# ReactiveBayes/RxInfer.jl

Hardware: AMD Instinct MI355X
Metric: node-message-updates/sec (d=4 LGSSM, T=100k, BP sweep with Bethe free energy) (higher is better)
Workload: dtype f64; 1 GPU; LGSSM d=4 dy=4 T=100000, 1024 independent chains per GPU (BASELINE config 2), 1 BP sweep + Bethe free energy per step; chain c drawn from numpy default_rng(42+c); chains_per_gpu=1024, T=100000, segments=128, segment_len=782

## Files before the change

rxinfer.jl_amd/csrc/engine.hpp:

```cpp
#pragma once
#include <hip/hip_runtime.h>

#include <cstdarg>
#include <cstdint>
#include <cstdio>
#include <initializer_list>
#include <string>
#include <vector>

#include "../../include/rxhip.h"
#include "lgssm_plan.hpp"
#include "tree_engine.hpp"

namespace rxhip {
struct LgssmVtbl;
struct DenseModel;
}
struct DenseTables;
using rxhip::DenseModel;
using rxhip::LgssmVtbl;

struct rxhip_engine_life {
    bool have_data = false;
    long long stream_k = 0;
// ... 118 lines not shown
        long long N = 0;
        int K = 0, KT = 0, materialize = 0, nblocks = 0, it = 0, iterations = 0, hist_cap = 0;
        int mvd = 0;
        int nq = 0;
        int hist_stride = 0;
        int state_size = 0;
        double *d_resp = nullptr, *d_par = nullptr, *d_drv = nullptr, *d_prior = nullptr, *d_init = nullptr,
               *d_partial = nullptr, *d_totals = nullptr, *d_hist = nullptr, *d_fe = nullptr;
    } g;
    bool dense = false;
    int nt = 0;
    double *d_scanm = nullptr, *d_fstart_m = nullptr, *d_beta_xi = nullptr, *d_vend = nullptr, *d_qtab = nullptr, *d_loc = nullptr, *d_bnd = nullptr;
    const int* d_canon = nullptr;
    int scan_sg = 1, scan_ng = 1;
    int agg_oc = 1, agg_kc = 1;
    double* d_aggpart = nullptr;
    bool fused = false;
    double *d_ftab = nullptr, *d_mtab = nullptr, *d_ntab = nullptr, *d_pos = nullptr, *d_fseg = nullptr;
    double fe_const = 0.0;
    double *d_gtab = nullptr, *d_segend = nullptr, *d_sblk = nullptr;
    int ck_log2 = 0;
    int sweep_waves_fwd = 1, sweep_waves_bwd = 1;
    long long nck = 0;
    double *d_amp = nullptr, *d_ainv = nullptr;
    int* d_ckfail = nullptr;
    hipEvent_t ev_tab0 = nullptr, ev_tab1 = nullptr;
    bool sequential = false;
    double* d_elemx = nullptr;
    double* h_io = nullptr;
    size_t h_io_bytes = 0;
    double* h_stream = nullptr;
    double* d_stream = nullptr;
    double *d_mu = nullptr, *d_nu = nullptr, *d_cx = nullptr, *d_cy_raw = nullptr;
    std::vector<double> h_mu, h_nu, h_cx, h_cy, h_offA, h_offB;
    std::vector<double> h_cx_const, h_cy_const;
    std::vector<int> h_offsm;
    int du = 0;
    std::vector<double> h_Bu;
    std::vector<char> h_umask;
    bool off_chain = false;
    double* d_off_chain = nullptr;
    std::vector<double> h_user;
    double* d_user = nullptr;
    int* d_step_model = nullptr;
    bool split = false, split_ready = false;
    int m_dpad = 0, m_nt = 0;
    int m_sg = 0, m_ng = 0;
// ... 131 lines not shown
```

rxinfer.jl_amd/csrc/launch_tables.hpp:

```cpp
#pragma once
#include <hip/hip_runtime.h>

#include <cstdlib>

#include "lgssm_kernels.hpp"
#include "predict_kernels.hpp"
#include "noise_kernels.hpp"
#ifndef RXHIP_LAUNCH_LGSSM_ONLY
#include "dense_kernels.hpp"
#include "dense_tab_kernels.hpp"
#include "dense_mseg_kernels.hpp"
#include "dense_split_kernels.hpp"
#include "dense8_kernels.hpp"
#endif

#ifndef RXHIP_TAB_SAME_TOL
#define RXHIP_TAB_SAME_TOL 5e-15
#endif

namespace rxhip {

struct SweepArgs {
    bool rev;
    int bnd;
    bool write_cov;
    int y_ring;
    int waves;
};
struct LgssmVtbl {
    int d, dy;
    int cst_size, tab_size, agg_size;
    int oA, oP, oLOBS, oG, oQI, oC0, oM1, oV1, oHF;
    int tK, tU;
    int aPI, aC, aJ, aCI, aX, aJJ;
    int scan_size, sM1, sM2, sVB, sN1, sN2, sLB;
    int f0_size, fK, fU, fSI, pos_size, pPI, pJ, pC, fs_size, fsA1, fsA2, fsW, mt_row;
    void (*forward0)(const Params&, const double*, bool, bool, int, hipStream_t);
    void (*time_tables)(const TimeTabParams&, hipStream_t);
    void (*fe_seg)(const Params&, hipStream_t);
    int gt_row, se_size;
    void (*smooth_tables)(const SmoothTabParams&, const double*, hipStream_t);
    void (*backward_sh)(const Params&, const double*, const double* gtab, const double* segend, const SweepArgs&, hipStream_t);
    void (*boundary_scan_tab)(const Params&, const double*, bool, hipStream_t);
    void (*seg_aggregate)(const Params&, const double*, bool, hipStream_t);
    int ex_size;
    void (*seg_elements)(const Params&, hipStream_t);
    void (*boundary_scan)(const Params&, const double*, bool, bool, hipStream_t);
    void (*forward)(const Params&, const double*, bool, bool, hipStream_t);
    void (*backward)(const Params&, const double*, bool, hipStream_t);
    void (*forecast)(const PredictParams&, hipStream_t);
    void (*predict)(const PredictParams&, hipStream_t);
    void (*joint)(const PredictParams&, hipStream_t);
    void (*stream_step)(const StreamParams&, hipStream_t);
    void (*small_sweep)(const Params&, const double*, bool, hipStream_t);
    int noise_prior_size;
    void (*noise_reset)(const NoiseParams&, hipStream_t);
    void (*noise_update)(const NoiseParams&, hipStream_t);
};
void lgssm_vtbls_d1(LgssmVtbl* out);
void lgssm_vtbls_d2(LgssmVtbl* out);
void lgssm_vtbls_d3(LgssmVtbl* out);
void lgssm_vtbls_d4(LgssmVtbl* out);

// ... 38 lines not shown
```

rxinfer.jl_amd/csrc/lgssm_kernels.hpp:

```cpp
#pragma once
#include <hip/hip_runtime.h>
#include <stdint.h>

namespace rxhip {

constexpr int ST_NOT_POSDEF = 1;
constexpr int ST_NONFINITE = 2;
__device__ __forceinline__ void lds_barrier() {
    __builtin_amdgcn_fence(__ATOMIC_RELEASE, "workgroup", "local");
    __builtin_amdgcn_s_barrier();
    __builtin_amdgcn_fence(__ATOMIC_ACQUIRE, "workgroup", "local");
}
__device__ __forceinline__ bool is_finite(double x) { return (__double2hiint(x) & 0x7ff00000) != 0x7ff00000; }

#ifndef RXHIP_NT_STORES
#define RXHIP_NT_STORES 0
#endif
typedef double rx_d2v __attribute__((ext_vector_type(2)));
__device__ __forceinline__ void stream_store(double2* p, double a, double b) {
#if RXHIP_NT_STORES
    rx_d2v v = {a, b};
    __builtin_nontemporal_store(v, reinterpret_cast<rx_d2v*>(p));
#else
    *p = make_double2(a, b);
// ... 152 lines not shown
    double* beta;
    double* fe_part;
    double* fe_chain;
    double* fe_total;
    int iteration;
    int filter;
    double fe_scale;
    int* status;
    int masked;
    const double* ftab;
    const double* mtab;
    const double* ntab;
    const double* fseg;
    double fe_const;
    double* elemx;
    const int* step_model;
    const double* noise_B;
    double* noise_part;
    int skip_marginals;
    int tinv_records;
    int elem_full;
    int ck_log2;
    long long nck;
    const double* ainv;
};


__device__ __forceinline__ double rcp_pos(double x) {
    double r = __builtin_amdgcn_rcp(x);
    double e = __builtin_fma(-x, r, 1.0);
    r = __builtin_fma(r, e, r);
    e = __builtin_fma(-x, r, 1.0);
    r = __builtin_fma(r, e, r);
    return r;
}

template <int D>
__device__ __forceinline__ bool spd_inv(const Sym<D>& a, Sym<D>& out, double& det) {
    double L[D][D], W[D][D], r[D];
    bool ok = true;
    det = 1.0;
#pragma unroll
    for (int j = 0; j < D; ++j) {
        double s = a(j, j);
#pragma unroll
        for (int k = 0; k < j; ++k) s -= W[j][k] * L[j][k];
        ok = ok && (s > 0.0);
// ... 2416 lines not shown
        __syncthreads();
        fe_few_body(p, small_lds);
    }
}
static __global__ void __launch_bounds__(256) k_fe_total(Params p, const double* block_part, int nblocks) {
    __shared__ double sh[256];
    double local = 0.0;
    for (int b = threadIdx.x; b < nblocks; b += 256) local += block_part[b];
    sh[threadIdx.x] = local;
    __syncthreads();
    for (int w = 128; w > 0; w >>= 1) {
        if ((int)threadIdx.x < w) sh[threadIdx.x] += sh[threadIdx.x + w];
        __syncthreads();
    }
    if (threadIdx.x == 0) p.fe_total[p.iteration] = sh[0];
}


template <int D>
struct SmoothTab {
    static constexpr int E = 0, F = D * D, G = 2 * D * D, VS = 3 * D * D;
    static constexpr int SIZE = 4 * D * D;
};
template <int D>
struct SegEndTab {
    static constexpr int H1 = 0, H2 = D * D;
    static constexpr int SIZE = 2 * D * D;
};
constexpr int SMOOTH_LB = 32;
template <int D>
struct SmoothBlk {
    static constexpr int GA = 0, CA = D * D, VE = 2 * D * D;
    static constexpr int SIZE = 3 * D * D;
};
struct SmoothTabParams {
    long long T, L;
    int S;
    const double* vtab;
    const double* ntab;
    const double* scan;
    double* gtab;
    double* segend;
    double* blk;
    int* status;
    int rev;
    double* amp;
    double* ainv;
    int* ckfail;
};
constexpr double REV_AMP_LIMIT = 1.0e2;
__host__ __device__ inline long long smooth_blocks_per_segment(long long L) { return (L + SMOOTH_LB - 1) / SMOOTH_LB; }

template <int D>
__device__ __forceinline__ void congruence(const double (&G)[D][D], const double (&V)[D][D], const double* C, double (&out)[D][D]) {
    double H[D][D];
#pragma unroll
    for (int a = 0; a < D; ++a)
#pragma unroll
        for (int b = 0; b < D; ++b) {
            double acc = 0.0;
#pragma unroll
            for (int k = 0; k < D; ++k) acc += G[a][k] * V[k][b];
            H[a][b] = acc;
        }
#pragma unroll
    for (int a = 0; a < D; ++a)
#pragma unroll
        for (int b = 0; b <= a; ++b) {
            double acc = C[a * D + b];
#pragma unroll
// ... 122 lines not shown
#pragma unroll
    for (int k = 0; k < NS; ++k) Vf.v[k] = q.vtab[t * NS + k];
    double AV[D][D], G[D][D], E[D][D];
    predict_cov<D>(CPtr{c.p + CL::A}, CPtr{c.p + CL::P}, Vf, AV, Vp);
    if (!spd_inv<D>(Vp, Lp, det)) atomicOr(q.status, ST_NOT_POSDEF);
#pragma unroll
    for (int a = 0; a < D; ++a)
#pragma unroll
        for (int b = 0; b < D; ++b) {
            double acc = 0.0;
#pragma unroll
            for (int k = 0; k < D; ++k) acc += AV[k][a] * Lp(k, b);
            G[a][b] = acc;
        }
#pragma unroll
    for (int a = 0; a < D; ++a)
#pragma unroll
        for (int b = 0; b < D; ++b) {
            double acc = (a == b) ? 1.0 : 0.0;
#pragma unroll
            for (int k = 0; k < D; ++k) acc -= G[a][k] * c[CL::A + k * D + b];
            E[a][b] = acc;
        }
    double* row = q.gtab + t * ST::SIZE;
    const double* N = q.ntab + t * MT;
    const bool at_start = t % q.L == 0;
    if (q.rev) {
        double Am[D][D], Ai[D][D], Mr[D][D];
#pragma unroll
        for (int a = 0; a < D; ++a)
#pragma unroll
            for (int b = 0; b < D; ++b) Am[a][b] = c[CL::A + a * D + b];
        const bool inv_ok = gen_inv<D>(Am, Ai);
#pragma unroll
        for (int a = 0; a < D; ++a)
#pragma unroll
            for (int b = 0; b < D; ++b) {
                double acc = 0.0;
#pragma unroll
                for (int k = 0; k < D; ++k) {
                    double phi = (k == b) ? 1.0 : 0.0;
#pragma unroll
                    for (int j = 0; j < D; ++j) phi += Vp(k, j) * c[CL::LOBS + sidx(j, b)];
                    acc += Ai[a][k] * phi;
                }
                Mr[a][b] = acc;
            }
        q.amp[t] = inv_ok ? spec_norm_bound<D>(Mr) : INFINITY;
        if (t == 0) {
#pragma unroll
            for (int a = 0; a < D; ++a)
#pragma unroll
                for (int b = 0; b < D; ++b) q.ainv[a * D + b] = Ai[a][b];
        }
    }
#pragma unroll
    for (int a = 0; a < D; ++a)
#pragma unroll
        for (int b = 0; b < D; ++b) {
            double f = 0.0;
            if (q.rev) f = Vp(a, b);
            else if (!at_start) {
#pragma unroll
                for (int k = 0; k < D; ++k) f += E[a][k] * N[k * D + b];
            }
            double cc = Vf(a, b);
#pragma unroll
            for (int k = 0; k < D; ++k) cc -= AV[k][a] * G[b][k];
            row[ST::E + a * D + b] = E[a][b];
            row[ST::F + a * D + b] = f;
            row[ST::G + a * D + b] = G[a][b];
            row[ST::VS + a * D + b] = cc;
        }
}

__device__ __forceinline__ bool smooth_block_range(const SmoothTabParams& q, long long id, long long& u0, long long& u1) {
    const long long nb = smooth_blocks_per_segment(q.L);
    const long long s = id / nb, j = id - s * nb;
    if (s >= q.S) return false;
    const long long tb = s * q.L;
    long long te = tb + q.L;
    if (te > q.T - 1) te = q.T - 1;
    u0 = tb + j * SMOOTH_LB;
    u1 = u0 + SMOOTH_LB;
    if (u1 > te) u1 = te;
    return u0 < u1;
}

template <int D>
__global__ void __launch_bounds__(64) k_smooth_tab_compose(SmoothTabParams q) {
    using ST = SmoothTab<D>;
    using SB = SmoothBlk<D>;
    const long long id = (long long)blockIdx.x * blockDim.x + threadIdx.x;
    long long u0, u1;
    if (!smooth_block_range(q, id, u0, u1)) return;
    if (q.rev) {
        double pk[3] = {1.0, 1.0, 1.0};
        int fail = 0;
        for (long long t = u0; t < u1; ++t) {
            const double a = q.amp[t];
            const double f = a >= 1.0 ? a : (a < 1.0 ? 1.0 : INFINITY);
#pragma unroll
            for (int k = 0; k < 3; ++k) {
                if (((t - u0) & ((8LL << k) - 1)) == 0) pk[k] = 1.0;
                else {
                    pk[k] *= f;
                    if (!(pk[k] <= REV_AMP_LIMIT)) fail |= 1 << k;
                }
            }
        }
        if (fail) atomicOr(q.ckfail, fail);
    }
    double Ga[D][D], Ca[D][D];
    {
// ... 21 lines not shown
                double acc = 0.0;
#pragma unroll
                for (int k = 0; k < D; ++k) acc += G[a][k] * Ga[k][b];
                Gn[a][b] = acc;
            }
#pragma unroll
        for (int a = 0; a < D; ++a)
#pragma unroll
            for (int b = 0; b < D; ++b) {
                Ga[a][b] = Gn[a][b];
                Ca[a][b] = Cn[a][b];
            }
    }
    double* o = q.blk + id * SB::SIZE;
#pragma unroll
    for (int a = 0; a < D; ++a)
#pragma unroll
        for (int b = 0; b < D; ++b) {
            o[SB::GA + a * D + b] = Ga[a][b];
            o[SB::CA + a * D + b] = Ca[a][b];
        }
}

template <int D>
__global__ void __launch_bounds__(64) k_smooth_tab_chain(SmoothTabParams q) {
    using SL = ScanLayout<D>;
    using ST = SmoothTab<D>;
    using SB = SmoothBlk<D>;
    constexpr int NS = Dim<D>::NS;
    const long long s = (long long)blockIdx.x * blockDim.x + threadIdx.x;
    if (s >= q.S) return;
    const long long tb = s * q.L;
    long long te = tb + q.L;
    if (te > q.T - 1) te = q.T - 1;
    bool ok = true;
    Sym<D> Vf, Vi, Ls, Vs;
    double det;
#pragma unroll
    for (int k = 0; k < NS; ++k) Vf.v[k] = q.vtab[te * NS + k];
    ok = spd_inv<D>(Vf, Vi, det) && ok;
#pragma unroll
    for (int k = 0; k < NS; ++k) Ls.v[k] = Vi.v[k] + q.scan[s * SL::SIZE + SL::LB + k];
    ok = spd_inv<D>(Ls, Vs, det) && ok;
    double* se = q.segend + s * SegEndTab<D>::SIZE;
    double V[D][D];
#pragma unroll
    for (int a = 0; a < D; ++a)
#pragma unroll
        for (int b = 0; b < D; ++b) {
            double acc = 0.0;
#pragma unroll
            for (int k = 0; k < D; ++k) acc += Vs(a, k) * Vi(k, b);
            se[SegEndTab<D>::H1 + a * D + b] = acc;
            se[SegEndTab<D>::H2 + a * D + b] = Vs(a, b);
            V[a][b] = Vs(a, b);
        }
    if (s == q.S - 1) {
        double* row = q.gtab + te * ST::SIZE;
#pragma unroll
        for (int a = 0; a < D; ++a)
#pragma unroll
            for (int b = 0; b < D; ++b) {
                row[ST::E + a * D + b] = row[ST::F + a * D + b] = row[ST::G + a * D + b] = 0.0;
                row[ST::VS + a * D + b] = Vs(a, b);
            }
    }
    const long long nb = smooth_blocks_per_segment(q.L);
    const long long used = te > tb ? (te - tb + SMOOTH_LB - 1) / SMOOTH_LB : 0;
    for (long long j = used - 1; j >= 0; --j) {
        double* o = q.blk + (s * nb + j) * SB::SIZE;
        double G[D][D], Vn[D][D];
#pragma unroll
        for (int a = 0; a < D; ++a)
#pragma unroll
            for (int b = 0; b < D; ++b) {
                o[SB::VE + a * D + b] = V[a][b];
                G[a][b] = o[SB::GA + a * D + b];
            }
        congruence<D>(G, V, o + SB::CA, Vn);
#pragma unroll
        for (int a = 0; a < D; ++a)
#pragma unroll
            for (int b = 0; b < D; ++b) V[a][b] = Vn[a][b];
    }
    if (!ok) atomicOr(q.status, ST_NOT_POSDEF);
}

template <int D>
__global__ void __launch_bounds__(64) k_smooth_tab_apply(SmoothTabParams q) {
    using ST = SmoothTab<D>;
    using SB = SmoothBlk<D>;
    const long long id = (long long)blockIdx.x * blockDim.x + threadIdx.x;
    long long u0, u1;
    if (!smooth_block_range(q, id, u0, u1)) return;
    double V[D][D];
    const double* o = q.blk + id * SB::SIZE;
#pragma unroll
    for (int a = 0; a < D; ++a)
#pragma unroll
        for (int b = 0; b < D; ++b) V[a][b] = o[SB::VE + a * D + b];
    for (long long t = u1 - 1; t >= u0; --t) {
        double* row = q.gtab + t * ST::SIZE;
        double G[D][D], Vn[D][D];
#pragma unroll
        for (int a = 0; a < D; ++a)
#pragma unroll
            for (int b = 0; b < D; ++b) G[a][b] = row[ST::G + a * D + b];
        congruence<D>(G, V, row + ST::VS, Vn);
#pragma unroll
        for (int a = 0; a < D; ++a)
#pragma unroll
            for (int b = 0; b < D; ++b) {
                V[a][b] = Vn[a][b];
// ... 232 lines not shown
    }
    boundary_chain<D, false>(p, chain - lane, (unsigned)lane, 0, (int)seg, lds, mseg);
#pragma unroll
    for (int i = 0; i < D; ++i) xb[i] = 0.0;
    boundary_chain<D, true>(p, chain - lane, (unsigned)lane, p.S - 1, p.S - 1 - (int)seg, lds, xb);
    const double* row = p.scan + seg * SL::SIZE;
    Sym<D> Vb, Lb;
#pragma unroll
    for (int i = 0; i < NS; ++i) {
        Vb.v[i] = row[SL::VB + i];
        Lb.v[i] = (seg == p.S - 1) ? 0.0 : row[SL::LB + i];
    }
    store_soa<D>(p.fstart, seg, p.n_chains, chain, mseg, Vb);
    store_soa<D>(p.beta, seg + 1, p.n_chains, chain, xb, Lb);
}

#ifndef RXHIP_Y_RING_DEPTH
#define RXHIP_Y_RING_DEPTH 4
#endif
constexpr int Y_RING_SHIPPED = RXHIP_Y_RING_DEPTH;
template <int D, int DY, int R, int W = 1>
__global__ void __launch_bounds__(64 * W) k_backward_sh_rev(Params p, const double* __restrict__ gtab, const double* __restrict__ segend,
                                                            const CstArg<CstLayout<D, DY>::SIZE> cb, const int bnd, const int write_cov) {
    using ST = SmoothTab<D>;
    using CL = CstLayout<D, DY>;
    constexpr int MP2 = DimM<D>::MP2;
    constexpr int MT = TimeTab<D>::MT;
    constexpr int U = 4;
    constexpr int RP = ST::SIZE / 2;
    constexpr int NPC = U * RP;
    static_assert(U % R == 0, "ring slots must be compile-time");
    static_assert(MT <= 64, "one lane per element of an N row");
    static_assert(D * D <= 64, "one lane per element of A⁻¹");
    __shared__ double2 tbuf[2][NPC];
    __shared__ double mtile_w[W][64 * D];
    __shared__ double bndbuf_w[W][2][BndStage<D>::N];
    __shared__ double ainv[D * D];
    __shared__ double nrow_w[W][MT];
    const int tid = threadIdx.x;
    const int wv = W > 1 ? __builtin_amdgcn_readfirstlane((int)(threadIdx.x >> 6)) : 0;
    const int lane = W > 1 ? (int)(threadIdx.x & 63) : (int)threadIdx.x;
    double (&mtile)[64 * D] = mtile_w[wv];
    double (&bndbuf)[2][BndStage<D>::N] = bndbuf_w[wv];
    double (&nrow)[MT] = nrow_w[wv];
    const long long g0 = ((long long)blockIdx.x * W + wv) * 64;
    const long long seg = g0 / p.n_chains;
    const long long chain0 = g0 - seg * p.n_chains;
    const long long chain = chain0 + lane;
    const long long len = seg_len(p, seg);
    const long long tb = seg * p.L, te = tb + len;
    const CPtr c{cb.v};
    const int lg = p.ck_log2;
    const long long K = 1LL << lg;
    auto load_ck = [&](long long t, double2 (&r)[MP2]) { load_filt_m_sh<D>(p, 1 + seg * p.nck + ((t - tb - 1) >> lg), chain, r); };
    double mseg[D], mf[D], ms[D];
    {
        double xb[D];
        if (bnd) boundary_in_sweep<D, DY>(p, c, seg, chain, lane, bnd == 2, bndbuf, mseg, xb);
        else {
            const double* q = p.fstart + (seg * Dim<D>::NP) * p.n_chains + chain;
            const double* bq = p.beta + ((seg + 1) * Dim<D>::NP) * p.n_chains + chain;
#pragma unroll
            for (int i = 0; i < D; ++i) {
                mseg[i] = q[i * p.n_chains];
                xb[i] = bq[i * p.n_chains];
            }
        }
        if (len > 0) {
            double2 r[MP2];
            load_ck(te, r);
            sweep_filt_mean<D>(r, p.ntab + te * MT, mseg, mf);
        } else {
#pragma unroll
            for (int i = 0; i < D; ++i) mf[i] = mseg[i];
        }
        sweep_segment_end<D>(segend, seg, mf, xb, ms);
    }
    auto write_out = [&](long long t, const double* vs) { sweep_write_out<D>(p, mtile, lane, chain0, ms, t, vs, write_cov); };
    if (seg == p.S - 1) write_out(te, gtab + te * ST::SIZE + ST::VS);
    if (len <= 0) return;

    const rx_d2v* g2 = reinterpret_cast<const rx_d2v*>(gtab);
    LdsStream<NPC, W> ts(tid);
    auto chunk = [&](long long i0) {
        return [&, i0](int idx, rx_d2v& v) {
            idx = idx < NPC ? idx : NPC - 1;
            const long long r = i0 + idx / RP;
            v = g2[(te - 1 - (r < len ? r : len - 1)) * RP + idx % RP];
        };
    };
    ts.fetch(chunk(0));
    if (tid < D * D) ainv[tid] = p.ainv[tid];
    ts.stash(tbuf[0]);
    ts.publish();
    long long tc = tb + (((len - 1) >> lg) << lg);
    double2 rc[MP2];
    double nc;
    auto prefetch_ck = [&]() {
        const long long t = tc > tb ? tc : (tb + K < te ? tb + K : te);
        load_ck(t, rc);
        nc = p.ntab[t * MT + (lane < MT ? lane : MT - 1)];
    };
    prefetch_ck();
    double yr[R][DY];
    auto y_index = [&](long long i) { return te - (i < len ? i : len - 1); };
#pragma unroll
    for (int r = 0; r < R; ++r) load_y<DY>(p.y, y_index(r), p.n_chains, chain, yr[r]);
    auto step = [&](const int u, const long long i, const int b) __attribute__((always_inline)) {
        const long long t = te - 1 - i;
        const double* row = reinterpret_cast<const double*>(&tbuf[b][0]) + u * ST::SIZE;
        const double (&yb)[DY] = yr[u % R];
        double mfn[D];
        if (t == tb) {
#pragma unroll
            for (int k = 0; k < D; ++k) mfn[k] = mseg[k];
        } else if (t == tc) {
            if (lane < MT) nrow[lane] = nc;
            __builtin_amdgcn_fence(__ATOMIC_RELEASE, "wavefront");
            __builtin_amdgcn_wave_barrier();
            __builtin_amdgcn_fence(__ATOMIC_ACQUIRE, "wavefront");
            sweep_filt_mean<D>(rc, nrow, mseg, mfn);
            __builtin_amdgcn_fence(__ATOMIC_RELEASE, "wavefront");
            __builtin_amdgcn_wave_barrier();
            __builtin_amdgcn_sched_barrier(0);
            tc -= K;
            prefetch_ck();
        } else {
            double w[D], mp[D];
#pragma unroll
            for (int a = 0; a < D; ++a) {
                double s = 0.0;
#pragma unroll
                for (int k = 0; k < D; ++k) s += c[CL::LOBS + sidx(a, k)] * mf[k];
#pragma unroll
                for (int k = 0; k < DY; ++k) s -= c[CL::G + a * DY + k] * yb[k];
                w[a] = s;
            }
#pragma unroll
            for (int a = 0; a < D; ++a) {
                double s = mf[a];
#pragma unroll
                for (int k = 0; k < D; ++k) s += row[ST::F + a * D + k] * w[k];
                mp[a] = s;
            }
#pragma unroll
            for (int a = 0; a < D; ++a) {
                double s = 0.0;
#pragma unroll
                for (int k = 0; k < D; ++k) s += ainv[a * D + k] * mp[k];
                mfn[a] = s;
            }
        }
        __builtin_amdgcn_sched_barrier(0);
        load_y<DY>(p.y, y_index(i + R), p.n_chains, chain, yr[u % R]);
        double mn[D];
#pragma unroll
        for (int a = 0; a < D; ++a) {
            double s0 = 0.0, s1 = 0.0;
#pragma unroll
            for (int k = 0; k < D; ++k) {
                s0 += row[ST::E + a * D + k] * mfn[k];
                s1 += row[ST::G + a * D + k] * ms[k];
            }
            mn[a] = s0 + s1;
        }
#pragma unroll
        for (int a = 0; a < D; ++a) {
            ms[a] = mn[a];
            mf[a] = mfn[a];
        }
        write_out(t, row + ST::VS);
    };
    int b = 0;
    long long i0 = 0;
    for (; i0 + U <= len; i0 += U, b ^= 1) {
        ts.fetch(chunk(i0 + U));
#pragma unroll
        for (int u = 0; u < U; ++u) step(u, i0 + u, b);
        ts.flip(tbuf[b ^ 1]);
    }
#pragma unroll
    for (int u = 0; u < U - 1; ++u)
        if (i0 + u < len) step(u, i0 + u, b);
}

}
```

rxinfer.jl_amd/csrc/rxhip.hip:

```cpp
#include "../../include/rxhip.h"

#include <hip/hip_runtime.h>

#include <algorithm>
#include <cmath>
#include <mutex>
#include <set>
#include <cstdarg>
#include <cstdio>
#include <cstring>
#include <cstdlib>
#include <string>
#include <vector>

#include "launch_tables.hpp"
#include "gseq_kernels.hpp"
#include "drift_kernels.hpp"
#include "generic_kernels.hpp"
#include "engine.hpp"
#include "graph_lowering.hpp"
#include "model_envelope.hpp"

using namespace rxhip;
using plan::ScheduleHooks;
// ... 1969 lines not shown
        once_per_device(16 + nt_split, e->device, [nt_split] { (void)dense_vt(nt_split)->split_prepare(); });
        ap.plain(&e->d_dtab, sizeof(double) * T * 3 * D * D);
        ap.plain(&e->d_vlast, sizeof(double) * D * D);
        ap.plain(&e->d_vstab, sizeof(double) * T * Du * Du);
        ap.plain(&e->d_fe_const, sizeof(double) * 2 * Sg);
    }
    if ((st = arena_commit(e, ap))) return st;
    tr.mark("dense: work buffers");
    return RXHIP_OK;
}
static rxhip_status lanes_time_tables(rxhip_engine* e, bool rev_cand, int ck_forced) {
    const LgssmVtbl* vt = e->vt;
    TimeTabParams q{};
    q.T = e->T; q.L = e->L; q.pos = e->d_pos; q.scan = e->d_scan; q.mtab = e->d_mtab; q.ntab = e->d_ntab; q.vtab = e->d_vtab;
    q.status = e->d_status;
    HIPCHK(e, hipEventCreate(&e->ev_tab0));
    HIPCHK(e, hipEventCreate(&e->ev_tab1));
    HIPCHK(e, hipEventRecord(e->ev_tab0, e->stream));
    vt->time_tables(q, e->stream);
    if (e->d_gtab) {
        SmoothTabParams sq{};
        sq.T = e->T; sq.L = e->L; sq.S = e->S; sq.vtab = e->d_vtab; sq.ntab = e->d_ntab; sq.scan = e->d_scan;
        sq.gtab = e->d_gtab; sq.segend = e->d_segend; sq.blk = e->d_sblk; sq.status = e->d_status;
        sq.rev = rev_cand ? 1 : 0; sq.amp = e->d_amp; sq.ainv = e->d_ainv; sq.ckfail = e->d_ckfail;
        vt->smooth_tables(sq, e->h_cst0.data(), e->stream);
        if (rev_cand) {
            int ckfail = 0;
            HIPCHK(e, hipMemcpyAsync(&ckfail, e->d_ckfail, sizeof(int), hipMemcpyDeviceToHost, e->stream));
            HIPCHK(e, hipStreamSynchronize(e->stream));
            e->ck_log2 = 0;
            if (ck_forced) {
                while ((1 << e->ck_log2) < ck_forced) ++e->ck_log2;
            } else {
                for (int k = 2; k >= 0 && !e->ck_log2; --k)
                    if (!((ckfail >> k) & 1)) e->ck_log2 = 3 + k;
            }
            if (!e->ck_log2) {
                sq.rev = 0;
                vt->smooth_tables(sq, e->h_cst0.data(), e->stream);
            }
        }
    }
    HIPCHK(e, hipEventRecord(e->ev_tab1, e->stream));
    HIPCHK(e, hipGetLastError());
    return RXHIP_OK;
}
static rxhip_status create_lanes(rxhip_engine* e, const rxhip_lgssm_desc* ds) {
// ... 32 lines not shown
    }
    if (e->uniform && !scan.empty()) ap.upload(&e->d_scan, scan.data(), sizeof(double) * scan.size());
    const int ck_forced = e->hooks.mean_checkpoint;
    if (ck_forced && (ck_forced < 1 || ck_forced > 32 || (ck_forced & (ck_forced - 1))))
        return fail(e, RXHIP_ERR_BADARG, "RXHIP_MEAN_CHECKPOINT=%s: a power of two from 1 to 32", e->hooks.mean_checkpoint_text.s);
    if (e->hooks.y_ring != 0 && e->hooks.y_ring != 1)
        return fail(e, RXHIP_ERR_BADARG, "RXHIP_Y_RING: 1 (the depth-1 y ring of the reverse-filter sweep) or unset (depth %d)", Y_RING_SHIPPED);
    const int waves_forced = e->hooks.sweep_waves;
    if (waves_forced < 0)
        return fail(e, RXHIP_ERR_BADARG, "RXHIP_SWEEP_WAVES: 1, 2 or 4 (wavefronts per workgroup of the reverse-filter sweep kernels) or unset");
    if (waves_forced > 1 && !plan::sweep_waves_divide(e->n_chains, waves_forced))
        return fail(e, RXHIP_ERR_BADARG, "RXHIP_SWEEP_WAVES=%d: a workgroup of %d waves takes %d chains of one segment, which does not divide the batch of %lld",
                    waves_forced, waves_forced, 64 * waves_forced, (long long)e->n_chains);
    e->sweep_waves_fwd = plan::sweep_waves(e->n_chains, plan::SWEEP_WAVES_FORWARD, waves_forced);
    e->sweep_waves_bwd = plan::sweep_waves(e->n_chains, plan::SWEEP_WAVES_BACKWARD, waves_forced);
    const bool rev_cand = plan::rev_cand(e->fused, e->n_chains, e->d, e->dy, e->T, e->hooks);
    if (e->fused) {
        ap.upload(&e->d_ftab, ft.ftab.data(), sizeof(double) * ft.ftab.size());
        ap.upload(&e->d_pos, ft.pos.data(), sizeof(double) * ft.pos.size());
        ap.upload(&e->d_fseg, ft.fseg.data(), sizeof(double) * ft.fseg.size());
        ap.plain(&e->d_mtab, sizeof(double) * T * vt->mt_row);
        ap.plain(&e->d_ntab, sizeof(double) * T * vt->mt_row);
        if (plan::gtab_tables(e->n_chains, e->hooks)) {
            ap.plain(&e->d_gtab, sizeof(double) * T * vt->gt_row);
            ap.plain(&e->d_segend, sizeof(double) * Sg * vt->se_size);
            ap.plain(&e->d_sblk, sizeof(double) * Sg * (size_t)smooth_blocks_per_segment(e->L) * 3 * e->d * e->d);
        }
        if (rev_cand) {
            ap.plain(&e->d_amp, sizeof(double) * T);
            ap.zeroed(&e->d_ainv, sizeof(double) * e->d * e->d);
            ap.zeroed(&e->d_ckfail, sizeof(int));
        }
    }
    ap.zeroed_last(&e->d_status, sizeof(int));
    ap.zeroed(&e->d_fe_part, sizeof(double) * (Sg + 2) * C);
    e->fe_total_cap = 16;
    ap.zeroed(&e->d_fe_total, sizeof(double) * e->fe_total_cap);
    ap.plain(&e->d_fe_blocks, sizeof(double) * ((C + 63) / 64));
    if (e->uniform) {
        const size_t MP2 = ((size_t)e->d + 1) / 2;
        if (!rev_cand) ap.plain(&e->d_filt, sizeof(double) * T * MP2 * 2 * (((C + 63) / 64) * 64));
        ap.plain(&e->d_vtab, sizeof(double) * T * ((size_t)e->d * (e->d + 1) / 2));
    } else
        ap.plain(&e->d_filt, sizeof(double) * T * NP2 * 2 * (((C + 63) / 64) * 64));
    ap.plain_first(&e->d_mean, sizeof(double) * (size_t)e->Tout() * C * e->d);
    ap.plain_first(&e->d_cov, sizeof(double) * (size_t)e->Tout() * C * e->d * e->d);
    ap.plain_first(&e->d_fe_chain, sizeof(double) * C);
    ap.plain(&e->d_elem, sizeof(double) * Sg * 2 * e->d * C);
    if (e->sequential && e->S > 1) ap.plain(&e->d_elemx, sizeof(double) * Sg * vt->ex_size * C);
    ap.plain(&e->d_fstart, sizeof(double) * Sg * NP * C);
    ap.plain(&e->d_beta, sizeof(double) * (Sg + 1) * NP * C);
    if (sizeof(double) * T * C * e->dy <= ((size_t)64 << 20)) {
        ap.plain(&e->d_y, sizeof(double) * T * C * e->dy);
// ... 433 lines not shown
    pl.backward_sh = fused && e->d_gtab;
    pl.elements_pass = pl.family == RunFamily::Elements && e->d_elemx;
    pl.fe_slots = e->S + (e->noise ? 1 : 0);
    pl.fe_part = e->d_fe_part;
    if (mseg) {
        pl.fe_part = e->m_fe_part;
        pl.fe_slots = 2 * e->mS - 1 + (int)mseg_resid_slots(e->T, e->m_dpad, e->dy, e->m_stepm, e->m_models);
    }
    if (e->dense && !e->gseq && pl.info) pl.fe_slots = 2 * e->S - 1 + fe_resid_blocks(e->T, e->dpad, e->dyk);
    return pl;
}
static Params fill_params(const rxhip_engine* e, const RunPlan& pl) {
    Params p;
    p.T = e->T;
    p.n_chains = e->n_chains;
    p.S = e->S;
    p.L = e->L;
    p.n_models = e->n_models;
    p.y = e->d_y;
    p.filt = e->d_filt;
    p.nb64 = (e->n_chains + 63) / 64;
    p.ck_log2 = e->ck_log2;
    p.nck = e->nck;
    p.ainv = e->d_ainv;
    p.vtab = e->d_vtab;
    p.scan = e->d_scan;
    p.mean = e->d_mean;
    p.cov = e->d_cov;
    p.cst = e->d_cst;
    p.tab = e->d_tab;
    p.agg = e->d_agg;
    p.chain_model = e->d_chain_model;
    p.elem = e->d_elem;
    p.fstart = e->d_fstart;
    p.beta = e->d_beta;
    p.fe_part = e->d_fe_part;
    p.fe_chain = e->d_fe_chain;
    p.fe_total = e->d_fe_total;
    p.status = e->d_status;
    p.filter = pl.filter ? 1 : 0;
    p.masked = e->masked ? 1 : 0;
    p.step_model = e->d_step_model;
    p.elemx = e->d_elemx;
    p.noise_B = pl.noise_in_sweep ? e->n_B : nullptr;
    p.noise_part = pl.noise_in_sweep ? e->n_part : nullptr;
    p.elem_full = pl.elem_full ? 1 : 0;
    p.tinv_records = pl.tinv_records ? 1 : 0;
// ... 767 lines not shown
```

rxinfer.jl_amd/csrc/tu_lgssm.hip:

```cpp
#include <cstring>
#include <type_traits>

#define RXHIP_LAUNCH_LGSSM_ONLY
#include "launch_tables.hpp"

#ifndef RXHIP_TU_D
#error "compile with -DRXHIP_TU_D=1..4"
#endif

namespace rxhip {
namespace {

template <class F>
void pick(bool b, F&& f) {
    if (b) f(std::true_type{});
    else f(std::false_type{});
}
template <class F>
void pick_waves(int w, F&& f) {
    if (w == 4) f(std::integral_constant<int, 4>{});
    else if (w == 2) f(std::integral_constant<int, 2>{});
    else f(std::integral_constant<int, 1>{});
}

// ... 50 lines not shown
        else if (p.noise_part) hipLaunchKernelGGL((k_backward_noise<D, DY>), grid, dim3(64), 0, s, p);
        else if (p.tinv_records) hipLaunchKernelGGL((k_backward_tinv<D, DY>), grid, dim3(64), 0, s, p);
        else hipLaunchKernelGGL((k_backward<D, DY, false>), grid, dim3(64), 0, s, p, CstArg<1>{});
    }
    static void forward0(const Params& p, const double* hc, bool fe, bool ck, int waves, hipStream_t s) {
        const long long total = p.n_chains * (long long)p.S;
        pick(fe, [&](auto FE) {
            if (ck)
                pick_waves(waves, [&](auto W) {
                    hipLaunchKernelGGL((k_forward0_ck<D, DY, FE(), W()>), dim3((unsigned)(p.n_chains / (64 * W()) * p.S)), dim3(64 * W()), 0, s, p, carg(hc));
                });
            else hipLaunchKernelGGL((k_forward0<D, DY, FE()>), dim3(nblk(total, 64)), dim3(64), 0, s, p, carg(hc));
        });
    }
    static void time_tables(const TimeTabParams& q, hipStream_t s) {
        hipLaunchKernelGGL((k_time_tables<D>), dim3(nblk(q.T, 64)), dim3(64), 0, s, q);
    }
    static void fe_seg(const Params& p, hipStream_t s) {
        hipLaunchKernelGGL((k_fe_seg<D>), dim3(nblk(p.n_chains * (long long)p.S, 64)), dim3(64), 0, s, p);
    }
    static void smooth_tables(const SmoothTabParams& q, const double* hc, hipStream_t s) {
        const long long nblocks = (long long)q.S * smooth_blocks_per_segment(q.L);
        if (q.T > 1) hipLaunchKernelGGL((k_smooth_tab_steps<D, DY>), dim3(nblk(q.T - 1, 64)), dim3(64), 0, s, q, carg(hc));
        hipLaunchKernelGGL((k_smooth_tab_compose<D>), dim3(nblk(nblocks, 64)), dim3(64), 0, s, q);
        hipLaunchKernelGGL((k_smooth_tab_chain<D>), dim3(nblk(q.S, 64)), dim3(64), 0, s, q);
        hipLaunchKernelGGL((k_smooth_tab_apply<D>), dim3(nblk(nblocks, 64)), dim3(64), 0, s, q);
    }
    static void backward_sh(const Params& p, const double* hc, const double* gtab, const double* segend, const SweepArgs& a, hipStream_t s) {
        const int write_cov = a.write_cov ? 1 : 0;
        if (!a.rev) {
            hipLaunchKernelGGL((k_backward_sh<D>), dim3((unsigned)(p.n_chains / 64 * p.S)), dim3(64), 0, s, p, gtab, segend, write_cov);
            return;
        }
        pick_waves(a.waves, [&](auto W) {
            pick(a.y_ring == 1, [&](auto R1) {
                constexpr int R = R1() ? 1 : Y_RING_SHIPPED;
                hipLaunchKernelGGL((k_backward_sh_rev<D, DY, R, W()>), dim3((unsigned)(p.n_chains / (64 * W()) * p.S)), dim3(64 * W()), 0, s, p, gtab, segend,
                                   carg(hc), a.bnd, write_cov);
            });
        });
    }
    static void forecast(const PredictParams& p, hipStream_t s) {
        hipLaunchKernelGGL((k_forecast<D, DY>), dim3(nblk(p.n_chains, 64)), dim3(64), 0, s, p);
    }
    static void predict(const PredictParams& p, hipStream_t s) {
        const long long total = (p.T + p.H) * p.n_chains;
// ... 24 lines not shown
        hipLaunchKernelGGL((k_stream_step<D, DY>), dim3(nblk(p.n_chains, 64)), dim3(64), 0, s, p);
    }
    static LgssmVtbl vtbl() {
        using TL = TabLayout<D, DY>;
        using AL = AggLayout<D>;
        LgssmVtbl v;
        v.d = D; v.dy = DY;
        v.cst_size = CL::SIZE; v.tab_size = TL::SIZE; v.agg_size = AL::SIZE;
        v.oA = CL::A; v.oP = CL::P; v.oLOBS = CL::LOBS; v.oG = CL::G; v.oQI = CL::QI; v.oC0 = CL::C0;
        v.oM1 = CL::M1; v.oV1 = CL::V1; v.oHF = CL::HF;
        v.tK = TL::K; v.tU = TL::U;
        v.aPI = AL::PI; v.aC = AL::C; v.aJ = AL::J; v.aCI = AL::CI; v.aX = AL::X; v.aJJ = AL::JJ;
        using SL = ScanLayout<D>;
        v.scan_size = SL::SIZE; v.sM1 = SL::M1; v.sM2 = SL::M2; v.sVB = SL::VB; v.sN1 = SL::N1; v.sN2 = SL::N2; v.sLB = SL::LB;
        using FL = F0Layout<D, DY>;
        using PL = PosLayout<D>;
        using FS = FeSegLayout<D>;
        v.f0_size = FL::SIZE; v.fK = FL::K; v.fU = FL::U; v.fSI = FL::SI;
        v.pos_size = PL::SIZE; v.pPI = PL::PI; v.pJ = PL::J; v.pC = PL::C;
        v.fs_size = FS::SIZE; v.fsA1 = FS::A1; v.fsA2 = FS::A2; v.fsW = FS::W; v.mt_row = TimeTab<D>::MT;
        v.forward0 = &Launch::forward0;
        v.time_tables = &Launch::time_tables;
        v.fe_seg = &Launch::fe_seg;
        v.gt_row = SmoothTab<D>::SIZE; v.se_size = SegEndTab<D>::SIZE;
        v.smooth_tables = &Launch::smooth_tables;
        v.backward_sh = &Launch::backward_sh;
        v.boundary_scan_tab = &Launch::boundary_scan_tab;
        v.seg_aggregate = &Launch::seg_aggregate;
        v.ex_size = ElemX<D>::SIZE;
        v.seg_elements = &Launch::seg_elements;
        v.boundary_scan = &Launch::boundary_scan;
        v.forward = &Launch::forward;
        v.backward = &Launch::backward;
        v.forecast = &Launch::forecast;
        v.predict = &Launch::predict;
        v.joint = &Launch::joint;
        v.stream_step = &Launch::stream_step;
        v.small_sweep = &Launch::small_sweep;
        v.noise_prior_size = NoisePrior<DY>::SIZE;
        v.noise_reset = &Launch::noise_reset;
        v.noise_update = &Launch::noise_update;
        return v;
    }
};

}

// ... 11 lines not shown
```

Before: 285.8 billion rule-calls/s.

## Precompute per-step reverse filter matrices in smoothing table for backward sweep

In the reversed backward sweep, the per-step mean update (observation-weighted w, then F·w plus mf, then multiply by A⁻¹) is replaced by a precomputed per-time R matrix and S gain stored in a widened smoothing table row. The table builder now writes A⁻¹·(V·LOBS) and A⁻¹·(V·G) per step, and the backward kernel streams only the live pieces plus optional covariance pieces into LDS. This removes the shared A⁻¹ load and cuts per-chain arithmetic in the hot loop. In exchange the gtab rows grow and more table bytes are fetched per step, with a layout that skips unused pieces.

```diff
diff --git a/rxinfer.jl_amd/csrc/engine.hpp b/rxinfer.jl_amd/csrc/engine.hpp
--- a/rxinfer.jl_amd/csrc/engine.hpp
+++ b/rxinfer.jl_amd/csrc/engine.hpp
@@ -164,7 +164,7 @@
     int ck_log2 = 0;
     int sweep_waves_fwd = 1, sweep_waves_bwd = 1;
     long long nck = 0;
-    double *d_amp = nullptr, *d_ainv = nullptr;
+    double* d_amp = nullptr;
     int* d_ckfail = nullptr;
     hipEvent_t ev_tab0 = nullptr, ev_tab1 = nullptr;
     bool sequential = false;
diff --git a/rxinfer.jl_amd/csrc/launch_tables.hpp b/rxinfer.jl_amd/csrc/launch_tables.hpp
--- a/rxinfer.jl_amd/csrc/launch_tables.hpp
+++ b/rxinfer.jl_amd/csrc/launch_tables.hpp
@@ -38,7 +38,7 @@
     void (*forward0)(const Params&, const double*, bool, bool, int, hipStream_t);
     void (*time_tables)(const TimeTabParams&, hipStream_t);
     void (*fe_seg)(const Params&, hipStream_t);
-    int gt_row, se_size;
+    int gt_row, gt_row_rev, se_size;
     void (*smooth_tables)(const SmoothTabParams&, const double*, hipStream_t);
     void (*backward_sh)(const Params&, const double*, const double* gtab, const double* segend, const SweepArgs&, hipStream_t);
     void (*boundary_scan_tab)(const Params&, const double*, bool, hipStream_t);
diff --git a/rxinfer.jl_amd/csrc/lgssm_kernels.hpp b/rxinfer.jl_amd/csrc/lgssm_kernels.hpp
--- a/rxinfer.jl_amd/csrc/lgssm_kernels.hpp
+++ b/rxinfer.jl_amd/csrc/lgssm_kernels.hpp
@@ -198,7 +198,7 @@
     int elem_full;
     int ck_log2;
     long long nck;
-    const double* ainv;
+    const double* unused0;
 };
 
 
@@ -2661,6 +2661,19 @@
     static constexpr int E = 0, F = D * D, G = 2 * D * D, VS = 3 * D * D;
     static constexpr int SIZE = 4 * D * D;
 };
+template <int D, int DY>
+struct SmoothTabRev {
+    static constexpr int E = 0, R = D * D, F = R, G = 2 * D * D, VS = 3 * D * D, S = 4 * D * D;
+    static constexpr int SIZE = ((S + D * DY + 1) / 2) * 2;
+    static constexpr int RP = SIZE / 2;
+    static constexpr int V0 = (VS + 1) / 2, V1 = (VS + D * D) / 2;
+    static constexpr int SKIP = V1 > V0 ? V1 - V0 : 0;
+    static constexpr int RPL = RP - SKIP;
+    static constexpr int VP0 = VS / 2, NVP = (VS + D * D + 1) / 2 - VP0;
+    static constexpr int S_LIVE = S - 2 * SKIP;
+    static constexpr int VS_OFF = VS - 2 * VP0;
+    __host__ __device__ static constexpr int live_piece(int j) { return j < V0 ? j : j + SKIP; }
+};
 template <int D>
 struct SegEndTab {
     static constexpr int H1 = 0, H2 = D * D;
@@ -2684,7 +2697,7 @@
     int* status;
     int rev;
     double* amp;
-    double* ainv;
+    double* unused0;
     int* ckfail;
 };
 constexpr double REV_AMP_LIMIT = 1.0e2;
@@ -2853,11 +2866,14 @@
             for (int k = 0; k < D; ++k) acc -= G[a][k] * c[CL::A + k * D + b];
             E[a][b] = acc;
         }
-    double* row = q.gtab + t * ST::SIZE;
+    using SR = SmoothTabRev<D, DY>;
+    static_assert(SR::E == ST::E && SR::F == ST::F && SR::G == ST::G && SR::VS == ST::VS, "one store for both rows");
+    double* row = q.gtab + t * (q.rev ? SR::SIZE : ST::SIZE);
     const double* N = q.ntab + t * MT;
     const bool at_start = t % q.L == 0;
+    double Rm[D][D];
     if (q.rev) {
-        double Am[D][D], Ai[D][D], Mr[D][D];
+        double Am[D][D], Ai[D][D];
 #pragma unroll
         for (int a = 0; a < D; ++a)
 #pragma unroll
@@ -2875,22 +2891,32 @@
                     for (int j = 0; j < D; ++j) phi += Vp(k, j) * c[CL::LOBS + sidx(j, b)];
                     acc += Ai[a][k] * phi;
                 }
-                Mr[a][b] = acc;
-            }
-        q.amp[t] = inv_ok ? spec_norm_bound<D>(Mr) : INFINITY;
-        if (t == 0) {
-#pragma unroll
-            for (int a = 0; a < D; ++a)
-#pragma unroll
-                for (int b = 0; b < D; ++b) q.ainv[a * D + b] = Ai[a][b];
-        }
+                Rm[a][b] = acc;
+            }
+        q.amp[t] = inv_ok ? spec_norm_bound<D>(Rm) : INFINITY;
+#pragma unroll
+        for (int a = 0; a < D; ++a)
+#pragma unroll
+            for (int j = 0; j < DY; ++j) {
+                double acc = 0.0;
+#pragma unroll
+                for (int k = 0; k < D; ++k) {
+                    double psi = 0.0;
+#pragma unroll
+                    for (int i = 0; i < D; ++i) psi += Vp(k, i) * c[CL::G + i * DY + j];
+                    acc += Ai[a][k] * psi;
+                }
+                row[SR::S + a * DY + j] = acc;
+            }
+#pragma unroll
+        for (int k = SR::S + D * DY; k < SR::SIZE; ++k) row[k] = 0.0;
     }
 #pragma unroll
     for (int a = 0; a < D; ++a)
 #pragma unroll
         for (int b = 0; b < D; ++b) {
             double f = 0.0;
-            if (q.rev) f = Vp(a, b);
+            if (q.rev) f = Rm[a][b];
             else if (!at_start) {
 #pragma unroll
                 for (int k = 0; k < D; ++k) f += E[a][k] * N[k * D + b];
@@ -2918,9 +2944,8 @@
     return u0 < u1;
 }
 
-template <int D>
+template <int D, class ST = SmoothTab<D>>
 __global__ void __launch_bounds__(64) k_smooth_tab_compose(SmoothTabParams q) {
-    using ST = SmoothTab<D>;
     using SB = SmoothBlk<D>;
     const long long id = (long long)blockIdx.x * blockDim.x + threadIdx.x;
     long long u0, u1;
@@ -2988,10 +3013,9 @@
         }
 }
 
-template <int D>
+template <int D, class ST = SmoothTab<D>>
 __global__ void __launch_bounds__(64) k_smooth_tab_chain(SmoothTabParams q) {
     using SL = ScanLayout<D>;
-    using ST = SmoothTab<D>;
     using SB = SmoothBlk<D>;
     constexpr int NS = Dim<D>::NS;
     const long long s = (long long)blockIdx.x * blockDim.x + threadIdx.x;
@@ -3030,6 +3054,8 @@
                 row[ST::E + a * D + b] = row[ST::F + a * D + b] = row[ST::G + a * D + b] = 0.0;
                 row[ST::VS + a * D + b] = Vs(a, b);
             }
+#pragma unroll
+        for (int k = 4 * D * D; k < ST::SIZE; ++k) row[k] = 0.0;
     }
     const long long nb = smooth_blocks_per_segment(q.L);
     const long long used = te > tb ? (te - tb + SMOOTH_LB - 1) / SMOOTH_LB : 0;
@@ -3052,9 +3078,8 @@
     if (!ok) atomicOr(q.status, ST_NOT_POSDEF);
 }
 
-template <int D>
+template <int D, class ST = SmoothTab<D>>
 __global__ void __launch_bounds__(64) k_smooth_tab_apply(SmoothTabParams q) {
-    using ST = SmoothTab<D>;
     using SB = SmoothBlk<D>;
     const long long id = (long long)blockIdx.x * blockDim.x + threadIdx.x;
     long long u0, u1;
@@ -3333,20 +3358,19 @@
 template <int D, int DY, int R, int W = 1>
 __global__ void __launch_bounds__(64 * W) k_backward_sh_rev(Params p, const double* __restrict__ gtab, const double* __restrict__ segend,
                                                             const CstArg<CstLayout<D, DY>::SIZE> cb, const int bnd, const int write_cov) {
-    using ST = SmoothTab<D>;
-    using CL = CstLayout<D, DY>;
+    using ST = SmoothTabRev<D, DY>;
     constexpr int MP2 = DimM<D>::MP2;
     constexpr int MT = TimeTab<D>::MT;
     constexpr int U = 4;
-    constexpr int RP = ST::SIZE / 2;
-    constexpr int NPC = U * RP;
+    constexpr int RP = ST::RP;
+    constexpr int NPL = U * ST::RPL;
+    constexpr int NPC = NPL + U * ST::NVP;
+    constexpr int LROW = 2 * ST::RPL;
     static_assert(U % R == 0, "ring slots must be compile-time");
     static_assert(MT <= 64, "one lane per element of an N row");
-    static_assert(D * D <= 64, "one lane per element of A⁻¹");
     __shared__ double2 tbuf[2][NPC];
     __shared__ double mtile_w[W][64 * D];
     __shared__ double bndbuf_w[W][2][BndStage<D>::N];
-    __shared__ double ainv[D * D];
     __shared__ double nrow_w[W][MT];
     const int tid = threadIdx.x;
     const int wv = W > 1 ? __builtin_amdgcn_readfirstlane((int)(threadIdx.x >> 6)) : 0;
@@ -3393,15 +3417,20 @@
 
     const rx_d2v* g2 = reinterpret_cast<const rx_d2v*>(gtab);
     LdsStream<NPC, W> ts(tid);
+    ts.fetch([](const int, rx_d2v& v) { v = rx_d2v{0.0, 0.0}; });
     auto chunk = [&](long long i0) {
         return [&, i0](int idx, rx_d2v& v) {
             idx = idx < NPC ? idx : NPC - 1;
-            const long long r = i0 + idx / RP;
-            v = g2[(te - 1 - (r < len ? r : len - 1)) * RP + idx % RP];
+            if (idx < NPL) {
+                const long long r = i0 + idx / ST::RPL;
+                v = g2[(te - 1 - (r < len ? r : len - 1)) * RP + ST::live_piece(idx % ST::RPL)];
+            } else if (write_cov) {
+                const long long r = i0 + (idx - NPL) / ST::NVP;
+                v = g2[(te - 1 - (r < len ? r : len - 1)) * RP + ST::VP0 + (idx - NPL) % ST::NVP];
+            }
         };
     };
     ts.fetch(chunk(0));
-    if (tid < D * D) ainv[tid] = p.ainv[tid];
     ts.stash(tbuf[0]);
     ts.publish();
     long long tc = tb + (((len - 1) >> lg) << lg);
@@ -3419,7 +3448,8 @@
     for (int r = 0; r < R; ++r) load_y<DY>(p.y, y_index(r), p.n_chains, chain, yr[r]);
     auto step = [&](const int u, const long long i, const int b) __attribute__((always_inline)) {
         const long long t = te - 1 - i;
-        const double* row = reinterpret_cast<const double*>(&tbuf[b][0]) + u * ST::SIZE;
+        const double* row = reinterpret_cast<const double*>(&tbuf[b][0]) + u * LROW;
+        const double* vs = reinterpret_cast<const double*>(&tbuf[b][NPL]) + u * (2 * ST::NVP) + ST::VS_OFF;
         const double (&yb)[DY] = yr[u % R];
         double mfn[D];
         if (t == tb) {
@@ -3437,28 +3467,13 @@
             tc -= K;
             prefetch_ck();
         } else {
-            double w[D], mp[D];
 #pragma unroll
             for (int a = 0; a < D; ++a) {
                 double s = 0.0;
 #pragma unroll
-                for (int k = 0; k < D; ++k) s += c[CL::LOBS + sidx(a, k)] * mf[k];
-#pragma unroll
-                for (int k = 0; k < DY; ++k) s -= c[CL::G + a * DY + k] * yb[k];
-                w[a] = s;
-            }
-#pragma unroll
-            for (int a = 0; a < D; ++a) {
-                double s = mf[a];
-#pragma unroll
-                for (int k = 0; k < D; ++k) s += row[ST::F + a * D + k] * w[k];
-                mp[a] = s;
-            }
-#pragma unroll
-            for (int a = 0; a < D; ++a) {
-                double s = 0.0;
-#pragma unroll
-                for (int k = 0; k < D; ++k) s += ainv[a * D + k] * mp[k];
+                for (int k = 0; k < D; ++k) s += row[ST::R + a * D + k] * mf[k];
+#pragma unroll
+                for (int k = 0; k < DY; ++k) s -= row[ST::S_LIVE + a * DY + k] * yb[k];
                 mfn[a] = s;
             }
         }
@@ -3480,7 +3495,7 @@
             ms[a] = mn[a];
             mf[a] = mfn[a];
         }
-        write_out(t, row + ST::VS);
+        write_out(t, vs);
     };
     int b = 0;
     long long i0 = 0;
diff --git a/rxinfer.jl_amd/csrc/rxhip.hip b/rxinfer.jl_amd/csrc/rxhip.hip
--- a/rxinfer.jl_amd/csrc/rxhip.hip
+++ b/rxinfer.jl_amd/csrc/rxhip.hip
@@ -2015,7 +2015,7 @@
         SmoothTabParams sq{};
         sq.T = e->T; sq.L = e->L; sq.S = e->S; sq.vtab = e->d_vtab; sq.ntab = e->d_ntab; sq.scan = e->d_scan;
         sq.gtab = e->d_gtab; sq.segend = e->d_segend; sq.blk = e->d_sblk; sq.status = e->d_status;
-        sq.rev = rev_cand ? 1 : 0; sq.amp = e->d_amp; sq.ainv = e->d_ainv; sq.ckfail = e->d_ckfail;
+        sq.rev = rev_cand ? 1 : 0; sq.amp = e->d_amp; sq.ckfail = e->d_ckfail;
         vt->smooth_tables(sq, e->h_cst0.data(), e->stream);
         if (rev_cand) {
             int ckfail = 0;
@@ -2094,13 +2094,12 @@
         ap.plain(&e->d_mtab, sizeof(double) * T * vt->mt_row);
         ap.plain(&e->d_ntab, sizeof(double) * T * vt->mt_row);
         if (plan::gtab_tables(e->n_chains, e->hooks)) {
-            ap.plain(&e->d_gtab, sizeof(double) * T * vt->gt_row);
+            ap.plain(&e->d_gtab, sizeof(double) * T * (rev_cand ? vt->gt_row_rev : vt->gt_row));
             ap.plain(&e->d_segend, sizeof(double) * Sg * vt->se_size);
             ap.plain(&e->d_sblk, sizeof(double) * Sg * (size_t)smooth_blocks_per_segment(e->L) * 3 * e->d * e->d);
         }
         if (rev_cand) {
             ap.plain(&e->d_amp, sizeof(double) * T);
-            ap.zeroed(&e->d_ainv, sizeof(double) * e->d * e->d);
             ap.zeroed(&e->d_ckfail, sizeof(int));
         }
     }
@@ -2580,7 +2579,6 @@
     p.nb64 = (e->n_chains + 63) / 64;
     p.ck_log2 = e->ck_log2;
     p.nck = e->nck;
-    p.ainv = e->d_ainv;
     p.vtab = e->d_vtab;
     p.scan = e->d_scan;
     p.mean = e->d_mean;
diff --git a/rxinfer.jl_amd/csrc/tu_lgssm.hip b/rxinfer.jl_amd/csrc/tu_lgssm.hip
--- a/rxinfer.jl_amd/csrc/tu_lgssm.hip
+++ b/rxinfer.jl_amd/csrc/tu_lgssm.hip
@@ -96,6 +96,13 @@
     static void smooth_tables(const SmoothTabParams& q, const double* hc, hipStream_t s) {
         const long long nblocks = (long long)q.S * smooth_blocks_per_segment(q.L);
         if (q.T > 1) hipLaunchKernelGGL((k_smooth_tab_steps<D, DY>), dim3(nblk(q.T - 1, 64)), dim3(64), 0, s, q, carg(hc));
+        if (q.rev) {
+            using SR = SmoothTabRev<D, DY>;
+            hipLaunchKernelGGL((k_smooth_tab_compose<D, SR>), dim3(nblk(nblocks, 64)), dim3(64), 0, s, q);
+            hipLaunchKernelGGL((k_smooth_tab_chain<D, SR>), dim3(nblk(q.S, 64)), dim3(64), 0, s, q);
+            hipLaunchKernelGGL((k_smooth_tab_apply<D, SR>), dim3(nblk(nblocks, 64)), dim3(64), 0, s, q);
+            return;
+        }
         hipLaunchKernelGGL((k_smooth_tab_compose<D>), dim3(nblk(nblocks, 64)), dim3(64), 0, s, q);
         hipLaunchKernelGGL((k_smooth_tab_chain<D>), dim3(nblk(q.S, 64)), dim3(64), 0, s, q);
         hipLaunchKernelGGL((k_smooth_tab_apply<D>), dim3(nblk(nblocks, 64)), dim3(64), 0, s, q);
@@ -166,7 +173,7 @@
         v.forward0 = &Launch::forward0;
         v.time_tables = &Launch::time_tables;
         v.fe_seg = &Launch::fe_seg;
-        v.gt_row = SmoothTab<D>::SIZE; v.se_size = SegEndTab<D>::SIZE;
+        v.gt_row = SmoothTab<D>::SIZE; v.gt_row_rev = SmoothTabRev<D, DY>::SIZE; v.se_size = SegEndTab<D>::SIZE;
         v.smooth_tables = &Launch::smooth_tables;
         v.backward_sh = &Launch::backward_sh;
         v.boundary_scan_tab = &Launch::boundary_scan_tab;
```

Result: no change. 288.0 billion rule-calls/s (median of 2 runs) (+0.8%).
